# tjjones6/Computational-Fluid-Dynamics

Measured on AMD Instinct MI355X. Metric: Poisson MLUPS + steps/sec, cavity 4096² @1/2/4/8 GPU; % HBM roofline, higher is better.
Workload: dtype f64

## Files before the change

### computational-fluid-dynamics_amd/cfd_amd/_lib.py

```python
from __future__ import annotations

import ctypes
import os

PKG_DIR = os.path.dirname(os.path.dirname(os.path.abspath(__file__)))
LIB_PATH = os.path.join(PKG_DIR, os.environ.get("CFD_AMD_LIB", "libcfd_amd.so"))

CFD_FIELD = {"p": 0, "src": 1, "us": 3, "vs": 4, "u": 5, "v": 6, "uc": 7, "vc": 8, "t": 9}
COMM_ID_BYTES = 128


class CfdParams(ctypes.Structure):
    _fields_ = [
        ("case_id", ctypes.c_int), ("nx", ctypes.c_int), ("ny", ctypes.c_int),
        ("length", ctypes.c_double), ("height", ctypes.c_double),
        ("re", ctypes.c_double), ("u_ref", ctypes.c_double), ("rho", ctypes.c_double), ("cfl", ctypes.c_double),
        ("final_time", ctypes.c_double),
        ("dx", ctypes.c_double), ("dy", ctypes.c_double), ("nu", ctypes.c_double), ("dt", ctypes.c_double),
        ("omega", ctypes.c_double),
        ("tol_factor", ctypes.c_double), ("abs_tol", ctypes.c_double),
        ("max_iters", ctypes.c_int), ("total_steps", ctypes.c_int),
        ("print_interval", ctypes.c_int), ("save_interval", ctypes.c_int),
        ("h_inlet", ctypes.c_double), ("step_x", ctypes.c_double),
        ("step_i", ctypes.c_int), ("inlet_jmax", ctypes.c_int),
# ... 24 lines not shown

class MgInfo(ctypes.Structure):
    _fields_ = [("levels", ctypes.c_int), ("coarse_nx", ctypes.c_int), ("coarse_ny", ctypes.c_int),
                ("coarse_sweeps", ctypes.c_int), ("solves", ctypes.c_longlong), ("cycles", ctypes.c_longlong),
                ("launches", ctypes.c_longlong), ("solve_ms", ctypes.c_double), ("fine_ms", ctypes.c_double)]


class StepInfo(ctypes.Structure):
    _fields_ = [("sor_iterations", ctypes.c_int), ("residual", ctypes.c_double)]


class Stats(ctypes.Structure):
    _fields_ = [("max_divergence", ctypes.c_double), ("avg_kinetic_energy", ctypes.c_double)]


class Timing(ctypes.Structure):
    _fields_ = [("poisson_ms", ctypes.c_double), ("poisson_launches", ctypes.c_longlong),
                ("poisson_cell_updates", ctypes.c_longlong), ("step_ms", ctypes.c_double),
                ("steps", ctypes.c_longlong), ("poisson_sweeps", ctypes.c_longlong),
                ("poisson_overlapped", ctypes.c_longlong), ("poisson_steady_ms", ctypes.c_double),
                ("poisson_steady_launches", ctypes.c_longlong),
                ("proof_fallbacks", ctypes.c_longlong), ("sor_kernel", ctypes.c_int),
                ("resident_timeouts", ctypes.c_longlong), ("seqsum_chunks", ctypes.c_longlong),
                ("seqsum_serial_chunks", ctypes.c_longlong), ("resident_segments", ctypes.c_longlong)]


_vp, _i, _d, _sz = ctypes.c_void_p, ctypes.c_int, ctypes.c_double, ctypes.c_size_t
_dp = ctypes.POINTER(ctypes.c_double)
_ip = ctypes.POINTER(ctypes.c_int)
SIGNATURES = {
    "cfd_abi_version": (_i, []),
    "cfd_last_error": (ctypes.c_char_p, []),
    "cfd_params_init": (_i, [_i, _d, _i, _i, _d, ctypes.POINTER(CfdParams)]),
    "cfd_create": (_vp, [ctypes.POINTER(CfdParams), _i, _i]),
    "cfd_create_rank": (_vp, [ctypes.POINTER(CfdParams), _i, _i, _i, _vp]),
    "cfd_destroy": (_i, [_vp]),
    "cfd_apply_bc": (_i, [_vp]),
    "cfd_apply_tentative_bc": (_i, [_vp]),
    "cfd_compute_tentative": (_i, [_vp]),
    "cfd_advance_temperature": (_i, [_vp]),
    "cfd_params_init_rb": (_i, [_d, _d, _i, _i, _d, ctypes.POINTER(CfdParams)]),
    "cfd_build_source": (_i, [_vp]),
    "cfd_solve_pressure": (_i, [_vp, ctypes.POINTER(StepInfo)]),
    "cfd_apply_correction": (_i, [_vp]),
    "cfd_step": (_i, [_vp, ctypes.POINTER(StepInfo)]),
    "cfd_run_steps": (_i, [_vp, _i, ctypes.POINTER(StepInfo)]),
    "cfd_compute_stats": (_i, [_vp, ctypes.POINTER(Stats)]),
# ... 53 lines not shown
```

### computational-fluid-dynamics_amd/csrc/lexw.hpp

```cpp
#pragma once

#include "kernels.hpp"

namespace cfd {

constexpr int LEXW_SHARDS = 8;
#ifndef CFD_LEXW_RAMP_EDGE_FULL
#define CFD_LEXW_RAMP_EDGE_FULL 1
#endif
#ifndef CFD_LEXW_W2
#define CFD_LEXW_W2 2
#endif
#ifndef CFD_LEXW_W3
#define CFD_LEXW_W3 2
#endif
#define CFD_LEXW_MIN_WAVES(NS) ((NS) <= 2 ? CFD_LEXW_W2 : CFD_LEXW_W3)

__host__ __device__ constexpr int lexw_twc(int ns) {
  return ns >= 6 ? 102 : ns == 5 ? 106 : ns == 4 ? 110 : PAIR_TWC;
}
__host__ __device__ constexpr int lexw_ch(int ns) { return ns >= 6 ? 12 : ns == 5 ? 10 : 8; }

#ifndef CFD_LEXW_LDS4
#define CFD_LEXW_LDS4 0
#endif
#ifndef CFD_LEXW_LDS_AHEAD
#define CFD_LEXW_LDS_AHEAD 1
#endif
__host__ __device__ constexpr bool lexw_lds(int kcase, int ns) {
  return kcase == CAVITY && (ns >= 5 || (ns == 4 && CFD_LEXW_LDS4));
}
__host__ __device__ constexpr int lexw_ring(int ns) { return ns <= 4 ? 8 : 16; }

constexpr int LEXW_RAMP_BANDS = 256;
struct LexRamp {
  int nb, th, row0;
  int wsplit;
  int xa, xn, xreach;
  unsigned band[LEXW_RAMP_BANDS];
};

__host__ __device__ inline int lexw_ramp_waves(const LexRamp& rp, int ctiles, int b, int ca, int cb, int o,
                                               int* ctile, int* half) {
  int sp[4], n = 0;
  if (rp.wsplit && ca == 0 && cb >= ca) sp[n++] = 0;
  if (rp.xn > 0 && rp.row0 + (b + 1) * rp.th + rp.xreach >= 0)
    for (int c = max(rp.xa, ca); c <= min(rp.xa + rp.xn - 1, cb); ++c)
      if (c != 0 && c != ctiles - 1) sp[n++] = c;
  if (rp.wsplit && cb == ctiles - 1 && cb > 0) sp[n++] = cb;
  int extra = 0;
  for (int q = 0; q < n; ++q) {
    const int at = sp[q] - ca + extra;
    if (o < at) break;
    if (o == at || o == at + 1) {
      *ctile = sp[q];
// ... 51 lines not shown
  }
  return true;
}

#define LX_SLOT(X) ((((ROT) + 4 - (X)) % 5 + 10) % 5)
#define LX_S10(X) ((((6 * (ROT) + 5 * (PAR)) % 10 + 9 - (X)) % 10 + 20) % 10)


struct LxDefer {
  double xp, ps;
  int k;
};

template <int NS, bool LR = false>
struct LexRun {
  double2 w[NS][5];
  double2 fr[LR ? 1 : 10];
  double2* ring;
  int rb;
  double2 np[5];
  double2 nf[5];
  unsigned long long mask;
  LxDefer d;
};

struct LexCtx {
  int H0;
  int K;
  double tol;
  double o2, o3, o4;
  int jg, jr1;
  double gz;
};

__device__ __forceinline__ double2 lx_ld(const WaveCtx<CAVITY>& x, const double* base, int R) {
  const int Rc = min(max(R, x.rmin), x.rmax);
  return *reinterpret_cast<const double2*>(base + (size_t)(Rc - x.g.row_lo) * (size_t)x.g.pitch + x.gic);
}

constexpr int LX_ACT = 1;
#ifndef CFD_LEXW_GROUPS
#define CFD_LEXW_GROUPS 1
#endif
#ifndef CFD_LEXW_ALLRC
#define CFD_LEXW_ALLRC 0
#endif
// ... 27 lines not shown
                                         double fc) {
  const double sum = (pE + pW) + (pN + pS) - fc * x.c.h2;
  const double oi = upd ? (top ? lc.o3 : lc.o4) : 0.0;
  double om, omm;
  if constexpr (EDGE) {
    const double ow = upd ? (top ? lc.o2 : lc.o3) : 0.0;
    om = cc.k == 2 ? oi : cc.k == 1 ? ow : 0.0;
    omm = (upd && cc.k != 0) ? x.c.one_m_omega : 1.0;
  } else {
    om = oi;
    omm = upd ? x.c.one_m_omega : 1.0;
  }
  return pc * omm + om * sum;
}

template <bool EDGE>
__device__ __forceinline__ double lx_res(const WaveCtx<CAVITY>& x, double eN, int i, double pc, double pW, double pE,
                                         double pS, double pN, double fc) {
  const double tE = (!EDGE || i < x.g.nx) ? (pE - pc) : 0.0;
  const double tW = (!EDGE || i > 1) ? (pW - pc) : 0.0;
  return fabs(x.c.idx2 * (tE + tW + (pN - pc) * eN + (pS - pc)) - fc);
}

template <int ROT, int JPAR, int COLOR, int MODE, bool EDGE, bool STORE, bool RES, bool UP = false>
__device__ __forceinline__ void lx_row(const WaveCtx<CAVITY>& x, const LexCtx& lc, const LxCol (&cc)[2],
                                       double2 (&W)[5], int j, int X, const LxAct& act, const double2& fc, int& exi) {
  double2& m = W[LX_SLOT(X)];
  const double2 nb = W[LX_SLOT(UP ? X - 1 : X + 1)], sb = W[LX_SLOT(UP ? X + 1 : X - 1)];
  const double2 old = m;
  const bool upd = j > x.rmin && j < x.rmax;
  const bool top = j == x.g.ny;
  constexpr bool A = ((JPAR ^ COLOR) & 1) == 0;
  if constexpr (A) {
    double nv = lx_upd<EDGE>(x, lc, upd, top, cc[0], m.x, dpp_from_left(m.y), m.y, sb.x, nb.x, fc.x);
    m.x = ((MODE & LX_ACT) && !act.a) ? m.x : nv;
  } else {
    double nv = lx_upd<EDGE>(x, lc, upd, top, cc[1], m.y, m.x, dpp_from_right(m.x), sb.y, nb.y, fc.y);
    m.y = ((MODE & LX_ACT) && !act.b) ? m.y : nv;
  }
  if (STORE && j >= x.y0 && j < x.y1 && x.out_lane) {
    double2* dst = reinterpret_cast<double2*>(x.pout + (size_t)(j - x.g.row_lo) * (size_t)x.g.pitch + x.gi);
    typedef double d2v __attribute__((ext_vector_type(2)));
    d2v mv = {m.x, m.y};
    __builtin_nontemporal_store(mv, reinterpret_cast<d2v*>(dst));
  }
  if constexpr (!RES || UP) return;
  const bool rrow = j >= x.y0 && j < x.y1 && j >= x.g.j0 && j <= x.g.j1;
  const double thr = rrow ? lc.tol : __builtin_huge_val();
  const double eN = top ? 0.0 : 1.0;
  bool ex;
  if constexpr (A) {
    ex = lx_res<EDGE>(x, eN, x.gi + 1, m.y, old.x, dpp_from_right(m.x), sb.y, nb.y, fc.y) > thr;
    if constexpr (EDGE) ex = ex && x.icol_b;
    if constexpr ((MODE & LX_ACT) != 0) ex = ex && act.c;
  } else {
    ex = lx_res<EDGE>(x, eN, x.gi, m.x, dpp_from_left(old.y), m.y, sb.x, nb.x, fc.x) > thr;
    if constexpr (EDGE) ex = ex && x.icol_a;
    if constexpr ((MODE & LX_ACT) != 0) ex = ex && act.b;
  }
  exi = ex ? 1 : exi;
  asm volatile("" : "+v"(exi));
}

struct LxoCol {
  int ka, kb;
  int sa, sb;
};
__device__ __forceinline__ int lxo_kind(const WaveCtx<CAVITY>& x, int i) {
  return (i < 0 || i > x.g.nx + 1) ? 0 : (i == 0) ? 1 : (i == x.g.nx + 1) ? 2 : 3;
}
// ... 199 lines not shown
template <int MODE, int T, int X, int NS>
constexpr bool lx_res_row() {
  return !(MODE & LX_SAMPLE) || (NS >= 5 ? (X - T + 2 * NS - 8 + 20) % 10 == 0 : T == X);
}
template <int MODE, int T, int NS>
constexpr bool lx_res_step() { return !(MODE & LX_SAMPLE) || NS >= 5 || (T >= 1 && T <= 2 * NS); }

template <int CASE>
struct LxCols {
  LxCol cc[2];
  LxoCol oc;
};

template <int T, int ROT, int PAR, int X, int NS, bool LR>
__device__ __forceinline__ double2 lx_fr(const LexRun<NS, LR>& s) {
  if constexpr (LR) {
    constexpr int D = lexw_ring(NS);
    return s.ring[((s.rb + (T + 9 - X + D)) & (D - 1)) * 64];
  } else {
    return s.fr[LX_S10(X)];
  }
}

template <int CASE, int S, int NS, int T, int ROT, int PAR, int MODE, bool EDGE, bool RC, bool UP = false, bool LR = false>
__device__ __forceinline__ void lx_sweeps(const WaveCtx<CAVITY>& x, const LexCtx& lc, const LexCtl& L,
                                          const LxCols<CASE>& cl, LexRun<NS, LR>& s, int R, const LxAct& act, int& exi,
                                          double2 f1 = make_double2(0.0, 0.0), double2 f2 = make_double2(0.0, 0.0)) {
  if constexpr (S < NS) {
    constexpr bool AH = LR && CFD_LEXW_LDS_AHEAD;
    if constexpr (!AH || S == 0) f1 = lx_fr<T, ROT, PAR, 2 * S + 1>(s), f2 = lx_fr<T, ROT, PAR, 2 * S + 2>(s);
    double2 g1 = f1, g2 = f2;
    if constexpr (AH && S + 1 < NS) g1 = lx_fr<T, ROT, PAR, 2 * S + 3>(s), g2 = lx_fr<T, ROT, PAR, 2 * S + 4>(s);
    constexpr int D = UP ? -1 : 1;
    if constexpr (CASE == CAVITY) {
      lx_row<ROT, PAR ^ 1, 0, MODE, EDGE, false, lx_res_row<MODE, T, 2 * S + 1, NS>(), UP>(
          x, lc, cl.cc, s.w[S], R + D * (2 * S + 1), 2 * S + 1, act, f1, exi);
      lx_row<ROT, PAR, 1, MODE, EDGE, S == NS - 1, lx_res_row<MODE, T, 2 * S + 2, NS>(), UP>(
          x, lc, cl.cc, s.w[S], R + D * (2 * S + 2), 2 * S + 2, act, f2, exi);
    } else {
      lxo_row<CASE, ROT, PAR ^ 1, 0, MODE, EDGE, RC, false, lx_res_row<MODE, T, 2 * S + 1, NS>(), S == 0, false, UP>(
          x, lc, L, cl.oc, s.w[S], R + D * (2 * S + 1), 2 * S + 1, act, f1, exi, s.d);
      double2* nxt = nullptr;
      if constexpr (S + 1 < NS && !UP) nxt = &s.w[S + 1][LX_SLOT(2 * S + 3)];
      lxo_row<CASE, ROT, PAR, 1, MODE, EDGE, RC, S == NS - 1, lx_res_row<MODE, T, 2 * S + 2, NS>(), false, S == NS - 1, UP>(
          x, lc, L, cl.oc, s.w[S], R + D * (2 * S + 2), 2 * S + 2, act, f2, exi, s.d, nxt);
    }
    if constexpr (S + 1 < NS) s.w[S + 1][LX_SLOT(2 * S + 2)] = s.w[S][LX_SLOT(2 * S + 2)];
    lx_sweeps<CASE, S + 1, NS, T, ROT, PAR, MODE, EDGE, RC, UP, LR>(x, lc, L, cl, s, R, act, exi, g1, g2);
  }
}

template <int CASE, int NS, int T, int ROT, int PAR, int MODE, bool EDGE, bool RC, bool UP = false, bool LR = false>
__device__ __forceinline__ void lx_step(const WaveCtx<CAVITY>& x, const LexCtx& lc, const LexCtl& L,
                                        const LxCols<CASE>& cl, LexRun<NS, LR>& s, int R, unsigned long long bit) {
  constexpr int D = UP ? -1 : 1;
  s.w[0][LX_SLOT(0)] = s.np[LX_SLOT(0)];
  if constexpr (LR) {
    constexpr int RD = lexw_ring(NS);
    s.ring[((s.rb + (T + 8 + RD)) & (RD - 1)) * 64] = s.nf[LX_SLOT(0)];
  } else {
    s.fr[LX_S10(1)] = s.nf[LX_SLOT(0)];
  }
  s.np[LX_SLOT(-4)] = lx_ld(x, x.pin, R - 4 * D);
  s.nf[LX_SLOT(-4)] = lx_ld(x, x.f, R - 3 * D);
  int exi = 0;
  const LxAct act = lx_act<MODE, CASE == BACKSTEP && EDGE && RC>(lc, x.gi, R);
  lx_sweeps<CASE, 0, NS, T, ROT, PAR, MODE, EDGE, RC, UP, LR>(x, lc, L, cl, s, R, act, exi);
  if constexpr (UP) return;
  if constexpr (!lx_res_step<MODE, T, NS>()) return;
  s.mask |= exi ? bit : 0ull;
}

__device__ __forceinline__ unsigned long long wave_or64(unsigned long long v) {
#pragma unroll
  for (int off = 32; off > 0; off >>= 1) {
    const unsigned lo = (unsigned)v, hi = (unsigned)(v >> 32);
    v |= (unsigned long long)(unsigned)__shfl_xor((int)lo, off, 64) |
         ((unsigned long long)(unsigned)__shfl_xor((int)hi, off, 64) << 32);
  }
  return v;
}

__device__ __forceinline__ void lexw_flush(const LexCtl& L, int sh, int q0, const unsigned long long (&b)[3], int len) {
  unsigned long long* G = L.bits + (size_t)sh * L.words;
#pragma unroll
  for (int c = 0; c < 3; ++c) {
    if (c * 64 >= len || b[c] == 0) continue;
    const int q = q0 + c * 64;
    const int w = q >> 6, o = q & 63;
    if (w < L.words) atomicOr(&G[w], b[c] << o);
    if (o && w + 1 < L.words) atomicOr(&G[w + 1], b[c] >> (64 - o));
  }
}

template <int NS>
__device__ __forceinline__ double2* lx_ring() {
  __shared__ double2 ring[4 * lexw_ring(NS) * 64];
  return ring;
}

template <int CASE, int NS, int MODE, bool EDGE, bool RC = false, bool UP = false>
__device__ __forceinline__ void lx_march(const WaveCtx<CAVITY>& x, const LexCtx& lc, const LexCtl& L, int y0, int y1,
                                         int c0, int lane, int shard) {
  static_assert(!UP || (!(MODE & LX_ACT) && !EDGE && !RC), "upward march: the unmasked, unchecked interior bands");
  constexpr int H = 2 * NS + 1;
  constexpr int D = UP ? -1 : 1;
  const int Rb0 = UP ? y0 - H : y1 - 1 + H;
  const int Rbeg = UP ? Rb0 - (Rb0 & 1) : Rb0 + (Rb0 & 1);
  const int nsteps = (y1 - y0) + 2 * H + (Rb0 & 1);
  constexpr bool LR = lexw_lds(CASE, NS);
  LexRun<NS, LR> s;
  const double2 z = make_double2(0.0, 0.0);
#pragma unroll
  for (int k = 0; k < 5; ++k)
#pragma unroll
    for (int q = 0; q < NS; ++q) s.w[q][k] = z;
  if constexpr (LR) {
    s.ring = lx_ring<NS>() + (threadIdx.x >> 6) * (lexw_ring(NS) * 64) + lane;
    s.rb = 0;
#pragma unroll
    for (int k = 0; k < lexw_ring(NS); ++k) s.ring[k * 64] = z;
  } else {
#pragma unroll
    for (int k = 0; k < 10; ++k) s.fr[k] = z;
  }
  {
    constexpr int ROT = 0;
#pragma unroll
    for (int q = 0; q < 4; ++q) {
      s.np[LX_SLOT(-q)] = lx_ld(x, x.pin, Rbeg - D * q);
      s.nf[LX_SLOT(-q)] = lx_ld(x, x.f, Rbeg - D * (q - 1));
    }
  }
  s.mask = 0ull;
  s.d = LxDefer{0.0, 0.0, -1};
  LxCols<CASE> cl;
  if constexpr (EDGE && CASE == CAVITY) cl.cc[0] = lx_col(x, x.gi), cl.cc[1] = lx_col(x, x.gi + 1);
  if constexpr (EDGE && CASE != CAVITY)
    cl.oc = LxoCol{lxo_kind(x, x.gi), lxo_kind(x, x.gi + 1), lxs_class(x, x.gi), lxs_class(x, x.gi + 1)};
  int R = Rbeg;
  if constexpr (UP) {
    for (int st = 0; st < nsteps; st += 10, R += 10) {
      lx_step<CASE, NS, 0, 0, 0, MODE, EDGE, RC, true>(x, lc, L, cl, s, R, 0ull);
      lx_step<CASE, NS, 1, 1, 1, MODE, EDGE, RC, true>(x, lc, L, cl, s, R + 1, 0ull);
      lx_step<CASE, NS, 2, 2, 0, MODE, EDGE, RC, true>(x, lc, L, cl, s, R + 2, 0ull);
      lx_step<CASE, NS, 3, 3, 1, MODE, EDGE, RC, true>(x, lc, L, cl, s, R + 3, 0ull);
      lx_step<CASE, NS, 4, 4, 0, MODE, EDGE, RC, true>(x, lc, L, cl, s, R + 4, 0ull);
      lx_step<CASE, NS, 5, 0, 1, MODE, EDGE, RC, true>(x, lc, L, cl, s, R + 5, 0ull);
      lx_step<CASE, NS, 6, 1, 0, MODE, EDGE, RC, true>(x, lc, L, cl, s, R + 6, 0ull);
      lx_step<CASE, NS, 7, 2, 1, MODE, EDGE, RC, true>(x, lc, L, cl, s, R + 7, 0ull);
      lx_step<CASE, NS, 8, 3, 0, MODE, EDGE, RC, true>(x, lc, L, cl, s, R + 8, 0ull);
      lx_step<CASE, NS, 9, 4, 1, MODE, EDGE, RC, true>(x, lc, L, cl, s, R + 9, 0ull);
      if constexpr (LR) s.rb = (s.rb + 10) & (lexw_ring(NS) - 1);
    }
    return;
  }
#define LX_BIT(T) ((((st + (T)) >> 1) < 64) ? (1ull << ((st + (T)) >> 1)) : 0ull)
  for (int st = 0; st < nsteps; st += 10, R -= 10) {
#if CFD_LEXW_GROUPS
    if constexpr (RC && !EDGE && CASE == CHANNEL) {
      if (R - 8 >= 2 && R - 8 > x.rmin && R + 2 * NS < lc.jg && R + 2 * NS < x.rmax) {
        lx_step<CASE, NS, 0, 0, 0, MODE, EDGE, false>(x, lc, L, cl, s, R, LX_BIT(0));
        lx_step<CASE, NS, 1, 1, 1, MODE, EDGE, false>(x, lc, L, cl, s, R - 1, LX_BIT(1));
        lx_step<CASE, NS, 2, 2, 0, MODE, EDGE, false>(x, lc, L, cl, s, R - 2, LX_BIT(2));
        lx_step<CASE, NS, 3, 3, 1, MODE, EDGE, false>(x, lc, L, cl, s, R - 3, LX_BIT(3));
        lx_step<CASE, NS, 4, 4, 0, MODE, EDGE, false>(x, lc, L, cl, s, R - 4, LX_BIT(4));
        lx_step<CASE, NS, 5, 0, 1, MODE, EDGE, false>(x, lc, L, cl, s, R - 5, LX_BIT(5));
        lx_step<CASE, NS, 6, 1, 0, MODE, EDGE, false>(x, lc, L, cl, s, R - 6, LX_BIT(6));
        lx_step<CASE, NS, 7, 2, 1, MODE, EDGE, false>(x, lc, L, cl, s, R - 7, LX_BIT(7));
        lx_step<CASE, NS, 8, 3, 0, MODE, EDGE, false>(x, lc, L, cl, s, R - 8, LX_BIT(8));
        lx_step<CASE, NS, 9, 4, 1, MODE, EDGE, false>(x, lc, L, cl, s, R - 9, LX_BIT(9));
        continue;
      }
    }
#endif
    lx_step<CASE, NS, 0, 0, 0, MODE, EDGE, RC>(x, lc, L, cl, s, R, LX_BIT(0));
    lx_step<CASE, NS, 1, 1, 1, MODE, EDGE, RC>(x, lc, L, cl, s, R - 1, LX_BIT(1));
    lx_step<CASE, NS, 2, 2, 0, MODE, EDGE, RC>(x, lc, L, cl, s, R - 2, LX_BIT(2));
    lx_step<CASE, NS, 3, 3, 1, MODE, EDGE, RC>(x, lc, L, cl, s, R - 3, LX_BIT(3));
    lx_step<CASE, NS, 4, 4, 0, MODE, EDGE, RC>(x, lc, L, cl, s, R - 4, LX_BIT(4));
    lx_step<CASE, NS, 5, 0, 1, MODE, EDGE, RC>(x, lc, L, cl, s, R - 5, LX_BIT(5));
    lx_step<CASE, NS, 6, 1, 0, MODE, EDGE, RC>(x, lc, L, cl, s, R - 6, LX_BIT(6));
    lx_step<CASE, NS, 7, 2, 1, MODE, EDGE, RC>(x, lc, L, cl, s, R - 7, LX_BIT(7));
    lx_step<CASE, NS, 8, 3, 0, MODE, EDGE, RC>(x, lc, L, cl, s, R - 8, LX_BIT(8));
    lx_step<CASE, NS, 9, 4, 1, MODE, EDGE, RC>(x, lc, L, cl, s, R - 9, LX_BIT(9));
    if constexpr (LR) s.rb = (s.rb + 10) & (lexw_ring(NS) - 1);
  }
#undef LX_BIT
  const unsigned long long m = x.out_lane ? s.mask : 0ull;
  const int sh = 63 - lane;
  const unsigned long long lo = m << sh, hi = sh ? (m >> (64 - sh)) : 0ull;
  unsigned long long b[3] = {wave_or64(lo), wave_or64(hi), 0ull};
  const int Bd0 = (lc.H0 - c0 - Rbeg - 2) / 2 + 1;
  if (lane == 0) lexw_flush(L, shard, Bd0 - 63 + L.kmax, b, 128);
}

__host__ __device__ inline void lexw_rows(const Geo& g, int H0, int K, int ns, int ct, int* lo, int* hi,
                                          bool open = false) {
  const int twc = lexw_twc(ns);
  if (!open) {
    const int cmin = max(ct * twc, 1), cmax = min(ct * twc + twc - 1, g.nx);
    *lo = max(g.j0, H0 - 2 * ns - 2 * (K - 1) - cmax);
    *hi = min(g.j1, H0 + 2 * ns - 1 - cmin);
  } else {
    const int cmin = max(ct * twc, 0), cmax = min(ct * twc + twc - 1, g.nx + 1);
    *lo = max(g.wj0, H0 - 2 * ns - 2 * (K - 1) - cmax - 2);
    *hi = min(g.wj1, H0 + 2 * ns - 1 - cmin);
  }
}

#ifndef CFD_LEXW_STAMPS
#define CFD_LEXW_STAMPS 0
#endif
#if CFD_LEXW_STAMPS
constexpr int LEXW_STAMP_LAUNCHES = 8192;
static __device__ unsigned long long lexw_stamp_buf[LEXW_STAMP_LAUNCHES * 8 * 3];
#ifndef LEXW_WSTAMP_L0
#define LEXW_WSTAMP_L0 1500
#endif
constexpr int LEXW_WSTAMP_N = 8, LEXW_WSTAMP_T = 4096;
static __device__ unsigned long long lexw_wstamp_buf[LEXW_WSTAMP_N * LEXW_WSTAMP_T * 4];
#endif

template <int CASE, int NS, bool RAMP, bool SAMPLE = false>
__global__ __launch_bounds__(256, RAMP ? 2 : CFD_LEXW_MIN_WAVES(NS)) void poisson_lexw_kernel(Geo g, Coef c, const double* __restrict__ pin,
                                                              double* __restrict__ pout, const double* __restrict__ f,
                                                              LexCtl L, int H0, int K, int ka, int kb, PairPlan pl,
                                                              int flags, LexRamp rp) {
  static_assert(CASE == CAVITY || CASE == CHANNEL || CASE == BACKSTEP, "reference-order march: case");
  constexpr bool OPEN = CASE != CAVITY;
  constexpr int CH = lexw_ch(NS);
// ... 106 lines not shown
  x.icol_a = gi >= 1 && gi <= g.nx;
  x.icol_b = gi + 1 >= 1 && gi + 1 <= g.nx;
  x.open_a = x.open_b = true;
  x.gic = min(max(gi, 0), g.pitch - 2);
  auto uni = [](double v) {
    return __hiloint2double(__builtin_amdgcn_readfirstlane(__double2hiint(v)),
                            __builtin_amdgcn_readfirstlane(__double2loint(v)));
  };
  LexCtx lc{H0, K, L.tol[0], uni(c.om_nc[2]), uni(c.om_nc[3]), uni(c.om_nc[4]),
            left ? c.inlet_jmax + 1 : g.ny + 1, left ? min(g.j1, c.inlet_jmax) : g.j1, left ? 0.0 : -0.0};
  if (left) x.rmax = min(x.rmax, c.inlet_jmax + 2);
  const int shard = bl & (LEXW_SHARDS - 1);
  const bool edge = !cols_in;
  constexpr int SM = SAMPLE ? LX_SAMPLE : 0;
#if CFD_LEXW_STAMPS
  long long t0_;
  asm volatile("s_memtime %0\n\ts_waitcnt lgkmcnt(0)" : "=s"(t0_)::"memory");
  int path_ = 0;
#define LX_PATH(v) (path_ = (v))
#else
#define LX_PATH(v) ((void)0)
#endif
  if constexpr (!OPEN) {
    if constexpr (RAMP) {
      const bool full = smax <= H0 - 2 && Hend <= smin + last;
      if (edge && full && CFD_LEXW_RAMP_EDGE_FULL) { LX_PATH(0); lx_march<CASE, NS, SM, true>(x, lc, L, y0, y1, c0, lane, shard); }
      else if (edge) { LX_PATH(0); lx_march<CASE, NS, LX_ACT | SM, true>(x, lc, L, y0, y1, c0, lane, shard); }
      else if (full && SAMPLE && up) { LX_PATH(1); lx_march<CASE, NS, SM, false, false, SAMPLE>(x, lc, L, y0, y1, c0, lane, shard); }
      else if (full) { LX_PATH(1); lx_march<CASE, NS, SM, false>(x, lc, L, y0, y1, c0, lane, shard); }
      else { LX_PATH(2); lx_march<CASE, NS, LX_ACT | SM, false>(x, lc, L, y0, y1, c0, lane, shard); }
    } else {
      if (edge) { LX_PATH(0); lx_march<CASE, NS, SM, true>(x, lc, L, y0, y1, c0, lane, shard); }
      else if (SAMPLE && up) { LX_PATH(4); lx_march<CASE, NS, SM, false, false, SAMPLE>(x, lc, L, y0, y1, c0, lane, shard); }
      else { LX_PATH(3); lx_march<CASE, NS, SM, false>(x, lc, L, y0, y1, c0, lane, shard); }
    }
  } else {
    bool rc = CFD_LEXW_ALLRC || !(y0 - H + 1 > x.rmin && y1 + H + 2 * NS < min(x.rmax, lc.jg));
    bool edge_ = edge;
    if (CASE == BACKSTEP && !left) {
      const int jb = c.inlet_jmax + 1, si = c.step_i;
      if (c0 >= 1 && c0 + 127 <= si - 1 && y0 - H - 1 >= jb + 1 && y1 + H + 2 * NS + 1 <= g.ny) return;
      if (y1 + H + 2 * NS + 1 >= jb - 1 && c0 <= si + 1) rc = edge_ = true;
    }
    const bool edge = edge_;
    if constexpr (RAMP) {
      const bool full = !rc && smax <= H0 - 2 && Hend <= smin + 2 * (K - 1);
      const bool efull = smax + 2 <= H0 - 2 && Hend <= smin + 2 * (K - 1);
      if (edge && efull && CFD_LEXW_RAMP_EDGE_FULL) {
        LX_PATH(0);
        lx_march<CASE, NS, SM, true, true>(x, lc, L, y0, y1, c0, lane, shard);
      } else if (edge) { LX_PATH(0); lx_march<CASE, NS, LX_ACT | SM, true, true>(x, lc, L, y0, y1, c0, lane, shard); }
      else if (full && SAMPLE && up) { LX_PATH(1); lx_march<CASE, NS, SM, false, false, SAMPLE>(x, lc, L, y0, y1, c0, lane, shard); }
      else if (full) { LX_PATH(1); lx_march<CASE, NS, SM, false, false>(x, lc, L, y0, y1, c0, lane, shard); }
      else if (rc && efull && CFD_LEXW_RAMP_EDGE_FULL) {
        LX_PATH(6);
// ... 95 lines not shown
```

### computational-fluid-dynamics_amd/csrc/solver.hip

```cpp
#include <algorithm>
#include <cmath>
#include <cstdlib>
#include <cstring>
#include <string>
#include <vector>

#include "internal.hpp"
#include "kernels.hpp"
#include "lexw.hpp"
#include "small.hpp"
#include "tile.hpp"
#include "resident.hpp"
#include "open.hpp"
#include "smlex.hpp"
#include "seqsum.hpp"
#include "mg.hpp"

#ifndef CFD_LEXW_WALL_SPLIT
#define CFD_LEXW_WALL_SPLIT 1
#endif

namespace cfd {

static thread_local std::string g_last_error;
void set_last_error(const std::string& m) { g_last_error = m; }

#define HIPC(x)                                                                                  \
// ... 942 lines not shown
    const int twc = lexw_twc(ns), ch = lexw_ch(ns), si = C.step_i;
    *xa = -1;
    *xn = 0;
    for (int ct = 1; ct + 1 < pl.ctiles; ++ct) {
      const int c0 = ct * twc - ch;
      const bool left = c0 + 127 <= si - 1 && lexw_left_class();
      if (!left && c0 <= si + 1) {
        if (*xa < 0) *xa = ct;
        *xn = ct - *xa + 1;
      }
    }
  }
  bool lexw_left_class() const { return P.case_id == CFD_BACKSTEP && lexw_left; }
  void lexw_presolid() {
    if (!lexw_left_class()) return;
    for (auto& s : S)
      for (int b : {0, 1}) {
        const int n = std::max(C.step_i, P.ny) + 1;
        step_presolid_kernel<<<(n + 255) / 256, 256, 0, st>>>(s.g, C, s.b[pbuf(b)]);
        check_launch("step_presolid");
      }
  }

  void launch_lexw(int ns, bool steady, bool sample, const PairPlan& pl, const Geo& g, const double* pin,
                   double* pout, const double* f, const LexCtl& L, int H0, int K, int ka, int kb, bool replay,
                   int waves) {
    const int fl = (replay ? 4 : 0) | (lexw_left_class() ? 8 : 0) | (lexw_updown ? 16 : 0);
    const int ne = pl.ctiles >= 2 ? 2 : 1;
    int ntiles = ne * (pl.nbe0 + pl.nbe1) + (pl.ctiles - ne) * (pl.nb0 + pl.nb1);
    LexRamp rp{};
    if (!steady) {
      int rl = 1 << 30, rh = -1;
      long long tot = 0;
      std::vector<std::pair<int, int>> rr(pl.ctiles);
      for (int c = 0; c < pl.ctiles; ++c) {
        lexw_rows(g, H0, K, ns, c, &rr[c].first, &rr[c].second, P.case_id != CFD_CAVITY);
        if (rr[c].second >= rr[c].first) {
          rl = std::min(rl, rr[c].first);
          rh = std::max(rh, rr[c].second);
          tot += rr[c].second - rr[c].first + 1;
        }
      }
      if (rh < rl) return;
      const int ex = lexw_extra(ns);
      rp.wsplit = CFD_LEXW_WALL_SPLIT;
      if (P.case_id == CFD_BACKSTEP && CFD_LEXW_XSPLIT > 1) {
// ... 36 lines not shown
      ntiles = build(th);
      while (th < pl.th && ntiles > waves) ntiles = build(th += 10);
      if (th > pl.th) ntiles = build(th = std::max(pl.th, (rh - rl) / LEXW_RAMP_BANDS + 1));
      if (pl.ctiles > 255 || ntiles >= 65536) throw Error(CFD_E_ARG, "lexicographic ordering: grid too wide");
    }
    PairPlan plx = pl;
    if (steady && P.case_id == CFD_BACKSTEP && CFD_LEXW_XSPLIT > 1 && pl.nb1 == 0 && pl.ctiles >= 3) {
      const int jb = C.inlet_jmax + 1;
      int xa, xn;
      lexw_cross_tiles(ns, pl, &xa, &xn);
      int xb = -1;
      for (int b = 0; b < pl.nb0 && xb < 0; ++b)
        if (std::min(pl.lo0 + (b + 1) * pl.th, pl.hi0) + 4 * ns + 4 >= jb) xb = b;
      if (xa >= 0 && xb >= 0) {
        plx.xa = xa;
        plx.xn = xn;
        plx.xb = xb;
        plx.xbn = pl.nb0 - xb;
        plx.xparts = CFD_LEXW_XSPLIT;
        ntiles += plx.xn * plx.xbn * (plx.xparts - 1);
      }
    }
    if (ntiles == 0) return;
    const dim3 grid((ntiles + 3) / 4);
#define CFD_LEXW_LAUNCH(CASE, NS, R, SM) \
  poisson_lexw_kernel<CASE, NS, R, SM><<<grid, 256, 0, st>>>(g, C, pin, pout, f, L, H0, K, ka, kb, plx, fl, rp)
    if (P.case_id == CFD_BACKSTEP && ns == 3) {
      if (sample) { if (steady) CFD_LEXW_LAUNCH(BACKSTEP, 3, false, true); else CFD_LEXW_LAUNCH(BACKSTEP, 3, true, true); }
      else { if (steady) CFD_LEXW_LAUNCH(BACKSTEP, 3, false, false); else CFD_LEXW_LAUNCH(BACKSTEP, 3, true, false); }
    } else if (P.case_id == CFD_BACKSTEP) {
      if (sample) { if (steady) CFD_LEXW_LAUNCH(BACKSTEP, 4, false, true); else CFD_LEXW_LAUNCH(BACKSTEP, 4, true, true); }
      else { if (steady) CFD_LEXW_LAUNCH(BACKSTEP, 4, false, false); else CFD_LEXW_LAUNCH(BACKSTEP, 4, true, false); }
    } else if (P.case_id == CFD_CHANNEL && ns == 3) {
      if (sample) { if (steady) CFD_LEXW_LAUNCH(CHANNEL, 3, false, true); else CFD_LEXW_LAUNCH(CHANNEL, 3, true, true); }
      else { if (steady) CFD_LEXW_LAUNCH(CHANNEL, 3, false, false); else CFD_LEXW_LAUNCH(CHANNEL, 3, true, false); }
    } else if (P.case_id == CFD_CHANNEL) {
      if (sample) { if (steady) CFD_LEXW_LAUNCH(CHANNEL, 4, false, true); else CFD_LEXW_LAUNCH(CHANNEL, 4, true, true); }
      else { if (steady) CFD_LEXW_LAUNCH(CHANNEL, 4, false, false); else CFD_LEXW_LAUNCH(CHANNEL, 4, true, false); }
    } else if (ns == 6) {
      if (sample) { if (steady) CFD_LEXW_LAUNCH(CAVITY, 6, false, true); else CFD_LEXW_LAUNCH(CAVITY, 6, true, true); }
      else { if (steady) CFD_LEXW_LAUNCH(CAVITY, 6, false, false); else CFD_LEXW_LAUNCH(CAVITY, 6, true, false); }
    } else if (ns == 5) {
      if (sample) { if (steady) CFD_LEXW_LAUNCH(CAVITY, 5, false, true); else CFD_LEXW_LAUNCH(CAVITY, 5, true, true); }
      else { if (steady) CFD_LEXW_LAUNCH(CAVITY, 5, false, false); else CFD_LEXW_LAUNCH(CAVITY, 5, true, false); }
    } else if (ns == 4) {
      if (sample) { if (steady) CFD_LEXW_LAUNCH(CAVITY, 4, false, true); else CFD_LEXW_LAUNCH(CAVITY, 4, true, true); }
// ... 1640 lines not shown
```

### include/cfd_amd.h

```cpp
#ifndef CFD_AMD_H
#define CFD_AMD_H

#include <stddef.h>

#ifdef __cplusplus
extern "C" {
#endif

#define CFD_AMD_ABI_VERSION 14

enum cfd_case { CFD_CAVITY = 0, CFD_CHANNEL = 1, CFD_BACKSTEP = 2, CFD_RAYLEIGH_BENARD = 3 };

enum cfd_field {
  CFD_FIELD_P = 0,
  CFD_FIELD_SRC = 1,
  CFD_FIELD_US = 3,
  CFD_FIELD_VS = 4,
  CFD_FIELD_U = 5,
  CFD_FIELD_V = 6,
  CFD_FIELD_UC = 7,
  CFD_FIELD_VC = 8,
  CFD_FIELD_T = 9
};

// ... 41 lines not shown
} cfd_step_info;

typedef struct cfd_stats {
  double max_divergence;
  double avg_kinetic_energy;
} cfd_stats;

typedef struct cfd_timing {
  double poisson_ms;
  long long poisson_launches;
  long long poisson_cell_updates;
  double step_ms;
  long long steps;
  long long poisson_sweeps;
  long long poisson_overlapped;
  double poisson_steady_ms;
  long long poisson_steady_launches;
  long long proof_fallbacks;
  int sor_kernel;
  long long resident_timeouts;
  long long seqsum_chunks;
  long long seqsum_serial_chunks;
  long long resident_segments;
} cfd_timing;

enum cfd_sor_kernel {
  CFD_SOR_NONE = 0,
  CFD_SOR_MARCH = 1,
  CFD_SOR_TILE = 2,
  CFD_SOR_SMALL = 3,
  CFD_SOR_LEXW = 4,
  CFD_SOR_LEX = 5,
  CFD_SOR_SMLEX = 6,
  CFD_SOR_RESIDENT = 7,
  CFD_SOR_MULTIGRID = 8
};

enum cfd_poisson_method {
  CFD_POISSON_SOR = 0,
  CFD_POISSON_MULTIGRID = 1,
  CFD_POISSON_MULTIGRID_OPEN = 2
};
typedef struct cfd_mg_options {
  int pre_sweeps, post_sweeps, max_cycles;
} cfd_mg_options;
int cfd_set_poisson_method(cfd_solver* s, int method, const cfd_mg_options* opt);
// ... 85 lines not shown
```

Baseline: 805,400.

## Add unchecked plain-interior path for lexw SOR march on cavity bands

Adds a specialised 'plain' variant of the lexicographic wavefront SOR march for cavity tiles whose rows and columns lie wholly inside the interior. There it drops the per-row boundary and range checks, replaces index-computed global loads and stores with running byte pointers stepped by the pitch, and skips the residual-threshold row test in the middle trips. The host classifies tiles with the same predicate and records a cached count of plain tiles in the timing struct. The cost is more template instantiations, which can add code size and register pressure, and correctness depends on the interior predicate being exact.

```diff
diff --git a/computational-fluid-dynamics_amd/cfd_amd/_lib.py b/computational-fluid-dynamics_amd/cfd_amd/_lib.py
--- a/computational-fluid-dynamics_amd/cfd_amd/_lib.py
+++ b/computational-fluid-dynamics_amd/cfd_amd/_lib.py
@@ -70,7 +70,8 @@
                 ("poisson_steady_launches", ctypes.c_longlong),
                 ("proof_fallbacks", ctypes.c_longlong), ("sor_kernel", ctypes.c_int),
                 ("resident_timeouts", ctypes.c_longlong), ("seqsum_chunks", ctypes.c_longlong),
-                ("seqsum_serial_chunks", ctypes.c_longlong), ("resident_segments", ctypes.c_longlong)]
+                ("seqsum_serial_chunks", ctypes.c_longlong), ("resident_segments", ctypes.c_longlong),
+                ("lexw_plain_tiles", ctypes.c_longlong)]
 
 
 _vp, _i, _d, _sz = ctypes.c_void_p, ctypes.c_int, ctypes.c_double, ctypes.c_size_t
diff --git a/computational-fluid-dynamics_amd/csrc/lexw.hpp b/computational-fluid-dynamics_amd/csrc/lexw.hpp
--- a/computational-fluid-dynamics_amd/csrc/lexw.hpp
+++ b/computational-fluid-dynamics_amd/csrc/lexw.hpp
@@ -31,6 +31,24 @@
   return kcase == CAVITY && (ns >= 5 || (ns == 4 && CFD_LEXW_LDS4));
 }
 __host__ __device__ constexpr int lexw_ring(int ns) { return ns <= 4 ? 8 : 16; }
+
+constexpr int LX_PL_ROWS = 1, LX_PL_STORE = 2, LX_PL_THR = 4;
+#ifndef CFD_LEXW_PLAIN
+#define CFD_LEXW_PLAIN 1
+#endif
+__host__ __device__ constexpr int lexw_plain_bits(int ns, bool sample) {
+  return (sample && ns >= 3 && (CFD_LEXW_PLAIN & LX_PL_ROWS)) ? CFD_LEXW_PLAIN : 0;
+}
+__host__ __device__ inline bool lexw_plain_band(int ns, int y0, int y1, bool up, int rmin, int rmax, int ny) {
+  const int H = 2 * ns + 1;
+  const int Rb0 = up ? y0 - H : y1 - 1 + H;
+  const int Rbeg = up ? Rb0 - (Rb0 & 1) : Rb0 + (Rb0 & 1);
+  const int nsteps = (y1 - y0) + 2 * H + (Rb0 & 1);
+  const int nt = (nsteps + 9) / 10 * 10;
+  const int lo = up ? Rbeg - 2 * ns : Rbeg - nt - 3;
+  const int hi = up ? Rbeg + nt + 3 : Rbeg + 2 * ns;
+  return lo >= max(rmin, 0) + 1 && hi <= min(rmax, ny) - 1;
+}
 
 constexpr int LEXW_RAMP_BANDS = 256;
 struct LexRamp {
@@ -128,6 +146,9 @@
   double2 nf[5];
   unsigned long long mask;
   LxDefer d;
+  const char *lp, *lf;
+  char* sp;
+  unsigned go, so;
 };
 
 struct LexCtx {
@@ -201,14 +222,17 @@
   return fabs(x.c.idx2 * (tE + tW + (pN - pc) * eN + (pS - pc)) - fc);
 }
 
-template <int ROT, int JPAR, int COLOR, int MODE, bool EDGE, bool STORE, bool RES, bool UP = false>
+template <int ROT, int JPAR, int COLOR, int MODE, bool EDGE, bool STORE, bool RES, bool UP = false, int PL = 0>
 __device__ __forceinline__ void lx_row(const WaveCtx<CAVITY>& x, const LexCtx& lc, const LxCol (&cc)[2],
-                                       double2 (&W)[5], int j, int X, const LxAct& act, const double2& fc, int& exi) {
+                                       double2 (&W)[5], int j, int X, const LxAct& act, const double2& fc, int& exi,
+                                       char* srow = nullptr) {
+  static_assert(!PL || (!EDGE && !(MODE & LX_ACT)), "unchecked rows: wholly active interior bands");
+  constexpr bool PLAIN = (PL & LX_PL_ROWS) != 0;
   double2& m = W[LX_SLOT(X)];
   const double2 nb = W[LX_SLOT(UP ? X - 1 : X + 1)], sb = W[LX_SLOT(UP ? X + 1 : X - 1)];
   const double2 old = m;
-  const bool upd = j > x.rmin && j < x.rmax;
-  const bool top = j == x.g.ny;
+  const bool upd = PLAIN || (j > x.rmin && j < x.rmax);
+  const bool top = !PLAIN && j == x.g.ny;
   constexpr bool A = ((JPAR ^ COLOR) & 1) == 0;
   if constexpr (A) {
     double nv = lx_upd<EDGE>(x, lc, upd, top, cc[0], m.x, dpp_from_left(m.y), m.y, sb.x, nb.x, fc.x);
@@ -217,14 +241,15 @@
     double nv = lx_upd<EDGE>(x, lc, upd, top, cc[1], m.y, m.x, dpp_from_right(m.x), sb.y, nb.y, fc.y);
     m.y = ((MODE & LX_ACT) && !act.b) ? m.y : nv;
   }
-  if (STORE && j >= x.y0 && j < x.y1 && x.out_lane) {
-    double2* dst = reinterpret_cast<double2*>(x.pout + (size_t)(j - x.g.row_lo) * (size_t)x.g.pitch + x.gi);
+  if (STORE && ((PL & LX_PL_STORE) || (j >= x.y0 && j < x.y1)) && x.out_lane) {
+    double2* dst = PLAIN ? reinterpret_cast<double2*>(srow)
+                         : reinterpret_cast<double2*>(x.pout + (size_t)(j - x.g.row_lo) * (size_t)x.g.pitch + x.gi);
     typedef double d2v __attribute__((ext_vector_type(2)));
     d2v mv = {m.x, m.y};
     __builtin_nontemporal_store(mv, reinterpret_cast<d2v*>(dst));
   }
   if constexpr (!RES || UP) return;
-  const bool rrow = j >= x.y0 && j < x.y1 && j >= x.g.j0 && j <= x.g.j1;
+  const bool rrow = (PL & LX_PL_THR) || (j >= x.y0 && j < x.y1 && j >= x.g.j0 && j <= x.g.j1);
   const double thr = rrow ? lc.tol : __builtin_huge_val();
   const double eN = top ? 0.0 : 1.0;
   bool ex;
@@ -470,7 +495,8 @@
   }
 }
 
-template <int CASE, int S, int NS, int T, int ROT, int PAR, int MODE, bool EDGE, bool RC, bool UP = false, bool LR = false>
+template <int CASE, int S, int NS, int T, int ROT, int PAR, int MODE, bool EDGE, bool RC, bool UP = false, int PL = 0,
+          bool LR = false>
 __device__ __forceinline__ void lx_sweeps(const WaveCtx<CAVITY>& x, const LexCtx& lc, const LexCtl& L,
                                           const LxCols<CASE>& cl, LexRun<NS, LR>& s, int R, const LxAct& act, int& exi,
                                           double2 f1 = make_double2(0.0, 0.0), double2 f2 = make_double2(0.0, 0.0)) {
@@ -481,10 +507,10 @@
     if constexpr (AH && S + 1 < NS) g1 = lx_fr<T, ROT, PAR, 2 * S + 3>(s), g2 = lx_fr<T, ROT, PAR, 2 * S + 4>(s);
     constexpr int D = UP ? -1 : 1;
     if constexpr (CASE == CAVITY) {
-      lx_row<ROT, PAR ^ 1, 0, MODE, EDGE, false, lx_res_row<MODE, T, 2 * S + 1, NS>(), UP>(
+      lx_row<ROT, PAR ^ 1, 0, MODE, EDGE, false, lx_res_row<MODE, T, 2 * S + 1, NS>(), UP, PL>(
           x, lc, cl.cc, s.w[S], R + D * (2 * S + 1), 2 * S + 1, act, f1, exi);
-      lx_row<ROT, PAR, 1, MODE, EDGE, S == NS - 1, lx_res_row<MODE, T, 2 * S + 2, NS>(), UP>(
-          x, lc, cl.cc, s.w[S], R + D * (2 * S + 2), 2 * S + 2, act, f2, exi);
+      lx_row<ROT, PAR, 1, MODE, EDGE, S == NS - 1, lx_res_row<MODE, T, 2 * S + 2, NS>(), UP, PL>(
+          x, lc, cl.cc, s.w[S], R + D * (2 * S + 2), 2 * S + 2, act, f2, exi, (PL & LX_PL_ROWS) ? s.sp + s.so : nullptr);
     } else {
       lxo_row<CASE, ROT, PAR ^ 1, 0, MODE, EDGE, RC, false, lx_res_row<MODE, T, 2 * S + 1, NS>(), S == 0, false, UP>(
           x, lc, L, cl.oc, s.w[S], R + D * (2 * S + 1), 2 * S + 1, act, f1, exi, s.d);
@@ -494,11 +520,12 @@
           x, lc, L, cl.oc, s.w[S], R + D * (2 * S + 2), 2 * S + 2, act, f2, exi, s.d, nxt);
     }
     if constexpr (S + 1 < NS) s.w[S + 1][LX_SLOT(2 * S + 2)] = s.w[S][LX_SLOT(2 * S + 2)];
-    lx_sweeps<CASE, S + 1, NS, T, ROT, PAR, MODE, EDGE, RC, UP, LR>(x, lc, L, cl, s, R, act, exi, g1, g2);
-  }
-}
-
-template <int CASE, int NS, int T, int ROT, int PAR, int MODE, bool EDGE, bool RC, bool UP = false, bool LR = false>
+    lx_sweeps<CASE, S + 1, NS, T, ROT, PAR, MODE, EDGE, RC, UP, PL, LR>(x, lc, L, cl, s, R, act, exi, g1, g2);
+  }
+}
+
+template <int CASE, int NS, int T, int ROT, int PAR, int MODE, bool EDGE, bool RC, bool UP = false, int PL = 0,
+          bool LR = false>
 __device__ __forceinline__ void lx_step(const WaveCtx<CAVITY>& x, const LexCtx& lc, const LexCtl& L,
                                         const LxCols<CASE>& cl, LexRun<NS, LR>& s, int R, unsigned long long bit) {
   constexpr int D = UP ? -1 : 1;
@@ -509,11 +536,20 @@
   } else {
     s.fr[LX_S10(1)] = s.nf[LX_SLOT(0)];
   }
-  s.np[LX_SLOT(-4)] = lx_ld(x, x.pin, R - 4 * D);
-  s.nf[LX_SLOT(-4)] = lx_ld(x, x.f, R - 3 * D);
+  if constexpr ((PL & LX_PL_ROWS) != 0) {
+    const ptrdiff_t ds = -(ptrdiff_t)D * (ptrdiff_t)x.g.pitch * (ptrdiff_t)sizeof(double);
+    s.np[LX_SLOT(-4)] = *reinterpret_cast<const double2*>(s.lp + s.go);
+    s.nf[LX_SLOT(-4)] = *reinterpret_cast<const double2*>(s.lf + s.go);
+    s.lp += ds;
+    s.lf += ds;
+  } else {
+    s.np[LX_SLOT(-4)] = lx_ld(x, x.pin, R - 4 * D);
+    s.nf[LX_SLOT(-4)] = lx_ld(x, x.f, R - 3 * D);
+  }
   int exi = 0;
   const LxAct act = lx_act<MODE, CASE == BACKSTEP && EDGE && RC>(lc, x.gi, R);
-  lx_sweeps<CASE, 0, NS, T, ROT, PAR, MODE, EDGE, RC, UP, LR>(x, lc, L, cl, s, R, act, exi);
+  lx_sweeps<CASE, 0, NS, T, ROT, PAR, MODE, EDGE, RC, UP, PL, LR>(x, lc, L, cl, s, R, act, exi);
+  if constexpr ((PL & LX_PL_ROWS) != 0) s.sp -= (ptrdiff_t)D * (ptrdiff_t)x.g.pitch * (ptrdiff_t)sizeof(double);
   if constexpr (UP) return;
   if constexpr (!lx_res_step<MODE, T, NS>()) return;
   s.mask |= exi ? bit : 0ull;
@@ -547,10 +583,12 @@
   return ring;
 }
 
-template <int CASE, int NS, int MODE, bool EDGE, bool RC = false, bool UP = false>
+template <int CASE, int NS, int MODE, bool EDGE, bool RC = false, bool UP = false, int PL = 0>
 __device__ __forceinline__ void lx_march(const WaveCtx<CAVITY>& x, const LexCtx& lc, const LexCtl& L, int y0, int y1,
                                          int c0, int lane, int shard) {
   static_assert(!UP || (!(MODE & LX_ACT) && !EDGE && !RC), "upward march: the unmasked, unchecked interior bands");
+  static_assert(!PL || ((PL & LX_PL_ROWS) && CASE == CAVITY && !EDGE && !(MODE & LX_ACT)), "unchecked bands: cavity");
+  constexpr int PLG = PL & LX_PL_ROWS, PLM = UP ? (PL & ~LX_PL_THR) : PL;
   constexpr int H = 2 * NS + 1;
   constexpr int D = UP ? -1 : 1;
   const int Rb0 = UP ? y0 - H : y1 - 1 + H;
@@ -572,7 +610,22 @@
 #pragma unroll
     for (int k = 0; k < 10; ++k) s.fr[k] = z;
   }
-  {
+  if constexpr (PL != 0) {
+    constexpr int ROT = 0;
+    const ptrdiff_t pb = (ptrdiff_t)x.g.pitch * (ptrdiff_t)sizeof(double);
+    s.go = (unsigned)x.gic * (unsigned)sizeof(double);
+    s.so = (unsigned)x.gi * (unsigned)sizeof(double);
+    s.lp = reinterpret_cast<const char*>(x.pin) + (ptrdiff_t)(Rbeg - x.g.row_lo) * pb;
+    s.lf = reinterpret_cast<const char*>(x.f) + (ptrdiff_t)(Rbeg + D - x.g.row_lo) * pb;
+    s.sp = reinterpret_cast<char*>(x.pout) + (ptrdiff_t)(Rbeg + D * 2 * NS - x.g.row_lo) * pb;
+#pragma unroll
+    for (int q = 0; q < 4; ++q) {
+      s.np[LX_SLOT(-q)] = *reinterpret_cast<const double2*>(s.lp + s.go);
+      s.nf[LX_SLOT(-q)] = *reinterpret_cast<const double2*>(s.lf + s.go);
+      s.lp -= D * pb;
+      s.lf -= D * pb;
+    }
+  } else {
     constexpr int ROT = 0;
 #pragma unroll
     for (int q = 0; q < 4; ++q) {
@@ -587,6 +640,29 @@
   if constexpr (EDGE && CASE != CAVITY)
     cl.oc = LxoCol{lxo_kind(x, x.gi), lxo_kind(x, x.gi + 1), lxs_class(x, x.gi), lxs_class(x, x.gi + 1)};
   int R = Rbeg;
+#define LX_TRIP(UPF, PLV, SG, BIT)                                                              \
+  lx_step<CASE, NS, 0, 0, 0, MODE, EDGE, RC, UPF, PLV>(x, lc, L, cl, s, R, BIT(0));             \
+  lx_step<CASE, NS, 1, 1, 1, MODE, EDGE, RC, UPF, PLV>(x, lc, L, cl, s, R SG 1, BIT(1));        \
+  lx_step<CASE, NS, 2, 2, 0, MODE, EDGE, RC, UPF, PLV>(x, lc, L, cl, s, R SG 2, BIT(2));        \
+  lx_step<CASE, NS, 3, 3, 1, MODE, EDGE, RC, UPF, PLV>(x, lc, L, cl, s, R SG 3, BIT(3));        \
+  lx_step<CASE, NS, 4, 4, 0, MODE, EDGE, RC, UPF, PLV>(x, lc, L, cl, s, R SG 4, BIT(4));        \
+  lx_step<CASE, NS, 5, 0, 1, MODE, EDGE, RC, UPF, PLV>(x, lc, L, cl, s, R SG 5, BIT(5));        \
+  lx_step<CASE, NS, 6, 1, 0, MODE, EDGE, RC, UPF, PLV>(x, lc, L, cl, s, R SG 6, BIT(6));        \
+  lx_step<CASE, NS, 7, 2, 1, MODE, EDGE, RC, UPF, PLV>(x, lc, L, cl, s, R SG 7, BIT(7));        \
+  lx_step<CASE, NS, 8, 3, 0, MODE, EDGE, RC, UPF, PLV>(x, lc, L, cl, s, R SG 8, BIT(8));        \
+  lx_step<CASE, NS, 9, 4, 1, MODE, EDGE, RC, UPF, PLV>(x, lc, L, cl, s, R SG 9, BIT(9))
+#define LX_NOBIT(T) 0ull
+  if constexpr (UP && PL != 0) {
+    for (int st = 0; st < nsteps; st += 10, R += 10) {
+      if (PLM != PLG && R - 2 * NS >= y0 && R - 2 * NS + 9 < y1) {
+        LX_TRIP(true, PLM, +, LX_NOBIT);
+      } else {
+        LX_TRIP(true, PLG, +, LX_NOBIT);
+      }
+      if constexpr (LR) s.rb = (s.rb + 10) & (lexw_ring(NS) - 1);
+    }
+    return;
+  }
   if constexpr (UP) {
     for (int st = 0; st < nsteps; st += 10, R += 10) {
       lx_step<CASE, NS, 0, 0, 0, MODE, EDGE, RC, true>(x, lc, L, cl, s, R, 0ull);
@@ -604,7 +680,18 @@
     return;
   }
 #define LX_BIT(T) ((((st + (T)) >> 1) < 64) ? (1ull << ((st + (T)) >> 1)) : 0ull)
-  for (int st = 0; st < nsteps; st += 10, R -= 10) {
+  for (int st = 0; PL != 0 && st < nsteps; st += 10, R -= 10) {
+    const int jt = R + 2 * NS;
+    const bool mid = (PLM & LX_PL_THR) ? (R - 8 >= max(y0, x.g.j0) && jt < y1 && jt <= x.g.j1)
+                                        : (jt - 9 >= y0 && jt < y1);
+    if (PLM != PLG && mid) {
+      LX_TRIP(false, PLM, -, LX_BIT);
+    } else {
+      LX_TRIP(false, PLG, -, LX_BIT);
+    }
+    if constexpr (LR) s.rb = (s.rb + 10) & (lexw_ring(NS) - 1);
+  }
+  for (int st = 0; PL == 0 && st < nsteps; st += 10, R -= 10) {
 #if CFD_LEXW_GROUPS
     if constexpr (RC && !EDGE && CASE == CHANNEL) {
       if (R - 8 >= 2 && R - 8 > x.rmin && R + 2 * NS < lc.jg && R + 2 * NS < x.rmax) {
@@ -635,6 +722,8 @@
     if constexpr (LR) s.rb = (s.rb + 10) & (lexw_ring(NS) - 1);
   }
 #undef LX_BIT
+#undef LX_NOBIT
+#undef LX_TRIP
   const unsigned long long m = x.out_lane ? s.mask : 0ull;
   const int sh = 63 - lane;
   const unsigned long long lo = m << sh, hi = sh ? (m >> (64 - sh)) : 0ull;
@@ -655,6 +744,22 @@
     *lo = max(g.wj0, H0 - 2 * ns - 2 * (K - 1) - cmax - 2);
     *hi = min(g.wj1, H0 + 2 * ns - 1 - cmin);
   }
+}
+
+__host__ __device__ inline bool lexw_plain_tile(const Geo& g, int ns, bool sample, bool ramp, int H0, int K, int ct,
+                                                int y0, int y1, bool up) {
+  if (!lexw_plain_bits(ns, sample) || y0 >= y1) return false;
+  const int H = 2 * ns + 1;
+  const int c0 = ct * lexw_twc(ns) - lexw_ch(ns);
+  const int rlo = max(max(y0 - H - 1, 1), g.row_lo);
+  const int rhi = min(min(y1 + H, g.ny), g.row_lo + g.nrows - 1);
+  const int clo = max(c0, 1), chi = min(c0 + 127, g.nx);
+  const int smin = clo + rlo, smax = chi + rhi;
+  const int Hend = H0 + 2 * ns - 1, last = 2 * (K - 1);
+  if (ramp && (smin > Hend || smax + last < H0 - 2 * ns)) return false;
+  if (clo != c0 || chi != c0 + 127) return false;
+  if (ramp && !(smax <= H0 - 2 && Hend <= smin + last)) return false;
+  return lexw_plain_band(ns, y0, y1, up, max(g.row_lo, 0), min(g.row_lo + g.nrows - 1, g.ny + 1), g.ny);
 }
 
 #ifndef CFD_LEXW_STAMPS
@@ -807,15 +912,21 @@
 #define LX_PATH(v) ((void)0)
 #endif
   if constexpr (!OPEN) {
+    constexpr int PLF = lexw_plain_bits(NS, SAMPLE);
+    const bool plain = PLF != 0 && !edge && lexw_plain_band(NS, y0, y1, SAMPLE && up, x.rmin, x.rmax, g.ny);
     if constexpr (RAMP) {
       const bool full = smax <= H0 - 2 && Hend <= smin + last;
       if (edge && full && CFD_LEXW_RAMP_EDGE_FULL) { LX_PATH(0); lx_march<CASE, NS, SM, true>(x, lc, L, y0, y1, c0, lane, shard); }
       else if (edge) { LX_PATH(0); lx_march<CASE, NS, LX_ACT | SM, true>(x, lc, L, y0, y1, c0, lane, shard); }
+      else if (full && plain && up) { LX_PATH(1); lx_march<CASE, NS, SM, false, false, SAMPLE, PLF>(x, lc, L, y0, y1, c0, lane, shard); }
+      else if (full && plain) { LX_PATH(1); lx_march<CASE, NS, SM, false, false, false, PLF>(x, lc, L, y0, y1, c0, lane, shard); }
       else if (full && SAMPLE && up) { LX_PATH(1); lx_march<CASE, NS, SM, false, false, SAMPLE>(x, lc, L, y0, y1, c0, lane, shard); }
       else if (full) { LX_PATH(1); lx_march<CASE, NS, SM, false>(x, lc, L, y0, y1, c0, lane, shard); }
       else { LX_PATH(2); lx_march<CASE, NS, LX_ACT | SM, false>(x, lc, L, y0, y1, c0, lane, shard); }
     } else {
       if (edge) { LX_PATH(0); lx_march<CASE, NS, SM, true>(x, lc, L, y0, y1, c0, lane, shard); }
+      else if (plain && up) { LX_PATH(4); lx_march<CASE, NS, SM, false, false, SAMPLE, PLF>(x, lc, L, y0, y1, c0, lane, shard); }
+      else if (plain) { LX_PATH(3); lx_march<CASE, NS, SM, false, false, false, PLF>(x, lc, L, y0, y1, c0, lane, shard); }
       else if (SAMPLE && up) { LX_PATH(4); lx_march<CASE, NS, SM, false, false, SAMPLE>(x, lc, L, y0, y1, c0, lane, shard); }
       else { LX_PATH(3); lx_march<CASE, NS, SM, false>(x, lc, L, y0, y1, c0, lane, shard); }
     }
diff --git a/computational-fluid-dynamics_amd/csrc/solver.hip b/computational-fluid-dynamics_amd/csrc/solver.hip
--- a/computational-fluid-dynamics_amd/csrc/solver.hip
+++ b/computational-fluid-dynamics_amd/csrc/solver.hip
@@ -3,6 +3,7 @@
 #include <cstdlib>
 #include <cstring>
 #include <string>
+#include <unordered_map>
 #include <vector>
 
 #include "internal.hpp"
@@ -991,6 +992,43 @@
       }
   }
 
+  std::unordered_map<std::string, int> plain_counts;
+  long long lexw_plain_count(int ns, bool steady, bool sample, const PairPlan& pl, const Geo& g, int H0, int K, int fl,
+                             const LexRamp& rp) {
+    if (!lexw_plain_bits(ns, sample)) return 0;
+    const int head[10] = {ns, steady, steady ? 0 : H0, steady ? 0 : K, fl, rp.th, rp.row0, rp.nb, 0, 0};
+    std::string key(reinterpret_cast<const char*>(head), sizeof(head));
+    key.append(reinterpret_cast<const char*>(&pl), sizeof(pl));
+    key.append(reinterpret_cast<const char*>(&g), sizeof(g));
+    const auto hit = plain_counts.find(key);
+    if (hit != plain_counts.end()) return hit->second;
+    const bool updown = (fl & 16) != 0;
+    int n = 0;
+    if (steady) {
+      const int nbi = pl.nb0 + pl.nb1;
+      for (int band = 0; band < nbi; ++band) {
+        const bool r0 = band < pl.nb0;
+        const int y0 = r0 ? pl.lo0 + band * pl.th : pl.lo1 + (band - pl.nb0) * pl.th;
+        const int y1 = std::min(y0 + pl.th, r0 ? pl.hi0 : pl.hi1);
+        for (int ct = 1; ct + 1 < pl.ctiles; ++ct)
+          n += lexw_plain_tile(g, ns, sample, false, H0, K, ct, y0, y1, (band & 1) && updown);
+      }
+    } else {
+      for (int b = 0; b < rp.nb; ++b) {
+        const int ca = (rp.band[b] >> 8) & 255, cb = rp.band[b] & 255;
+        for (int ct = std::max(ca, 1); ct <= std::min(cb, pl.ctiles - 2); ++ct) {
+          int rlo, rhi;
+          lexw_rows(g, H0, K, ns, ct, &rlo, &rhi, false);
+          const int y0 = std::max(rp.row0 + b * rp.th, rlo), y1 = std::min(rp.row0 + (b + 1) * rp.th, rhi + 1);
+          n += lexw_plain_tile(g, ns, sample, true, H0, K, ct, y0, y1, (b & 1) && updown);
+        }
+      }
+    }
+    if (plain_counts.size() >= 65536) plain_counts.clear();
+    plain_counts.emplace(std::move(key), n);
+    return n;
+  }
+
   void launch_lexw(int ns, bool steady, bool sample, const PairPlan& pl, const Geo& g, const double* pin,
                    double* pout, const double* f, const LexCtl& L, int H0, int K, int ka, int kb, bool replay,
                    int waves) {
@@ -1073,6 +1111,7 @@
       }
     }
     if (ntiles == 0) return;
+    if (P.case_id == CFD_CAVITY) T.lexw_plain_tiles += lexw_plain_count(ns, steady, sample, plx, g, H0, K, fl, rp);
     const dim3 grid((ntiles + 3) / 4);
 #define CFD_LEXW_LAUNCH(CASE, NS, R, SM) \
   poisson_lexw_kernel<CASE, NS, R, SM><<<grid, 256, 0, st>>>(g, C, pin, pout, f, L, H0, K, ka, kb, plx, fl, rp)
diff --git a/include/cfd_amd.h b/include/cfd_amd.h
--- a/include/cfd_amd.h
+++ b/include/cfd_amd.h
@@ -87,6 +87,7 @@
   long long seqsum_chunks;
   long long seqsum_serial_chunks;
   long long resident_segments;
+  long long lexw_plain_tiles;
 } cfd_timing;
 
 enum cfd_sor_kernel {
```

Measured after the change: 797,800. About the same (-0.9%).
